# e-c-k-e-r/tortoise-tts

Hardware: AMD Instinct MI355X
Metric: audio-sec/wall-sec (RTF^-1), 16 AR candidates x 80 DDIM steps (higher is better)
Workload: dtype bf16; 1 GPU; configs[1]: 1 utterance/GPU, 64 text tokens, 16 AR candidates x 250 mel tokens (KV-cached decode), latent pass on 16 candidates, 80 DDIM steps with cond-free guidance at T=1088 (11.6 s audio); candidates=16, ddim_steps=80, mel_frames=1088, parallelism=single GPU, small_models=False, vocoder_in_step=False

## Files before the change

### tortoise_tts_amd/csrc/norm.hip

```cpp
#include <stdint.h>

#include "ttk_common.h"
#include "ttk_kernels.h"

namespace ttk {

template <typename OT, int NI>
__global__ void k_layernorm(const float* x, int64_t ldx, int rows, int d, const float* g1, const float* b1,
							const float* g2, const float* b2, OT* out, int64_t ldo, int frag, float* out2, const int64_t* out2_idx, int64_t out2_stride, const int64_t* out2_base) {
	constexpr bool HOIST = NI <= 4;
	const int lane = threadIdx.x & 63;
	const int row = blockIdx.x * (blockDim.x >> 6) + (threadIdx.x >> 6);
	if (row >= rows) return;
	if (out2_base) out2 = (float*)(uintptr_t)out2_base[0];
	if (out2 && out2_idx) out2 += out2_idx[0] * out2_stride;
	const int nchunk = d / 4;
	float4 v[NI];
	float4 pg[HOIST ? 2 : 1][HOIST ? NI : 1], pb[HOIST ? 2 : 1][HOIST ? NI : 1];
#pragma unroll
	for (int i = 0; i < NI; ++i) {
		const int c = lane + 64 * i;
		v[i] = c < nchunk ? *(const float4*)(x + (int64_t)row * ldx + 4 * c) : make_float4(0, 0, 0, 0);
	}
	if (HOIST) {
#pragma unroll
		for (int i = 0; i < (HOIST ? NI : 0); ++i) {
			const int c = lane + 64 * i < nchunk ? lane + 64 * i : 0;
			pg[0][i] = *(const float4*)(g1 + 4 * c); pb[0][i] = *(const float4*)(b1 + 4 * c);
			if (g2) { pg[HOIST ? 1 : 0][i] = *(const float4*)(g2 + 4 * c); pb[HOIST ? 1 : 0][i] = *(const float4*)(b2 + 4 * c); }
		}
	}
#pragma unroll
	for (int pass = 0; pass < 2; ++pass) {
		if (pass == 1 && !g2) break;
		const float* g = pass ? g2 : g1;
		const float* b = pass ? b2 : b1;
		float sum = 0.f;
#pragma unroll
		for (int i = 0; i < NI; ++i) sum += v[i].x + v[i].y + v[i].z + v[i].w;
		const float mean = wave_sum(sum) / (float)d;
		float sq = 0.f;
#pragma unroll
		for (int i = 0; i < NI; ++i)
			if (lane + 64 * i < nchunk) {
				const float a0 = v[i].x - mean, a1 = v[i].y - mean, a2 = v[i].z - mean, a3 = v[i].w - mean;
				sq += a0 * a0 + a1 * a1 + a2 * a2 + a3 * a3;
			}
		const float rstd = rsqrtf(wave_sum(sq) / (float)d + 1e-5f);
#pragma unroll
		for (int i = 0; i < NI; ++i) {
			const int c = lane + 64 * i;
			if (c < nchunk) {
				const float4 gg = HOIST ? pg[HOIST ? pass : 0][HOIST ? i : 0] : *(const float4*)(g + 4 * c), bb = HOIST ? pb[HOIST ? pass : 0][HOIST ? i : 0] : *(const float4*)(b + 4 * c);
				v[i].x = (v[i].x - mean) * rstd * gg.x + bb.x;
				v[i].y = (v[i].y - mean) * rstd * gg.y + bb.y;
				v[i].z = (v[i].z - mean) * rstd * gg.z + bb.z;
				v[i].w = (v[i].w - mean) * rstd * gg.w + bb.w;
			}
		}
	}
#pragma unroll
	for (int i = 0; i < NI; ++i) {
		const int c = lane + 64 * i;
		if (c < nchunk) {
			const int n = 4 * c;
			OT* o = frag ? out + TTK_FRAG_INDEX(row, n, d / 32) : out + (int64_t)row * ldo + n;
			o[0] = (OT)v[i].x; o[1] = (OT)v[i].y; o[2] = (OT)v[i].z; o[3] = (OT)v[i].w;
			if (out2) *(float4*)(out2 + (int64_t)row * d + n) = v[i];
		}
	}
}

void launch_layernorm(int dt, const float* x, int64_t ldx, int rows, int d, const float* g1, const float* b1,
					  const float* g2, const float* b2, void* out, int64_t ldo, int out_f32, hipStream_t s, int frag, float* out2,
					  const int64_t* out2_idx, int64_t out2_stride, const int64_t* out2_base) {
	ProfScope prof(PROF_LAYERNORM, (double)rows * d * (4.0 + (out_f32 ? 4.0 : dtype_size(dt))), s);
	const int grid = (rows + 3) / 4;
#define LN_GO(OT, NI) hipLaunchKernelGGL((k_layernorm<OT, NI>), dim3(grid), dim3(256), 0, s, x, ldx, rows, d, g1, b1, g2, b2, (OT*)out, ldo, frag, out2, out2_idx, out2_stride, out2_base)
	if (out_f32 || dt == DT_F32) { if (d <= 1024) LN_GO(float, 4); else LN_GO(float, 16); }
	else if (dt == DT_F16) { if (d <= 1024) LN_GO(f16, 4); else LN_GO(f16, 16); }
	else { if (d <= 1024) LN_GO(bf16, 4); else LN_GO(bf16, 16); }
#undef LN_GO
}

__global__ __launch_bounds__(256) void k_gn_stats(const float* x, int T, int C, int rows_per_chunk, float* part, const int* tlen, const int* need) {
	const int g = blockIdx.x, b = blockIdx.y, ch = blockIdx.z, cpg = C / 32;
	if (need && !need[b]) return;
	const int Tl = tlen ? tlen[b] : T;
	const int t0 = ch * rows_per_chunk;
	if (t0 >= Tl) return;
	const int rows = min(rows_per_chunk, Tl - t0);
	const float* base = x + ((int64_t)b * T + t0) * C + g * cpg;
	const int n = rows * cpg;
	__shared__ float sh[4];
	float v[8];
	float sum = 0.f;
#pragma unroll
	for (int i = 0; i < 8; ++i) {
		const int e = threadIdx.x + 256 * i;
		const int t = e / cpg, c = e - t * cpg;
		v[i] = e < n ? base[(int64_t)t * C + c] : 0.f;
		sum += v[i];
	}
	sum = wave_sum(sum);
	if ((threadIdx.x & 63) == 0) sh[threadIdx.x >> 6] = sum;
	__syncthreads();
	const float mean = (sh[0] + sh[1] + sh[2] + sh[3]) / (float)n;
	__syncthreads();
	float sq = 0.f;
#pragma unroll
	for (int i = 0; i < 8; ++i)
		if (threadIdx.x + 256 * i < n) { const float d = v[i] - mean; sq += d * d; }
	sq = wave_sum(sq);
	if ((threadIdx.x & 63) == 0) sh[threadIdx.x >> 6] = sq;
	__syncthreads();
	if (threadIdx.x == 0) {
		float* o = part + (((int64_t)b * 32 + g) * gridDim.z + ch) * 3;
		o[0] = (float)n; o[1] = mean; o[2] = sh[0] + sh[1] + sh[2] + sh[3];
	}
}

int gn_rows_per_chunk(int C) { const int r = 2048 / (C / 32); return r < 1 ? 1 : r; }
int gn_num_chunks(int T, int C) { const int r = gn_rows_per_chunk(C); return (T + r - 1) / r; }

void launch_gn_stats(const float* x, int nb, int T, int C, float* part, hipStream_t s, const int* tlen, const int* need) {
	ProfScope prof(PROF_GN_STATS, 4.0 * nb * T * C, s);
	hipLaunchKernelGGL(k_gn_stats, dim3(32, nb, gn_num_chunks(T, C)), dim3(256), 0, s, x, T, C, gn_rows_per_chunk(C), part, tlen, need);
}

template <typename OT>
__global__ __launch_bounds__(256) void k_gn_apply(GnApplyParams p) {
	constexpr int GN_PASSES = 2;
	__shared__ float s_mean[32], s_rstd[32];
	TTK_WSTAMP(p.stamps, blockIdx.x, 0);
	const int c4n = p.C / 4;
	const int rpp = 256 / c4n;
	const int strip = rpp * GN_PASSES;
	const int strips = (p.Tout + strip - 1) / strip;
	const int b = blockIdx.x / strips, t0 = (blockIdx.x - b * strips) * strip;
	const int Tl = p.tlen ? p.tlen[b] : p.Tout;
	const int nch = p.tlen ? (Tl + p.chunk_rows - 1) / p.chunk_rows : p.nchunks;
	const int c = (threadIdx.x % c4n) * 4, rr = threadIdx.x / c4n;
	float4 xv[GN_PASSES];
#pragma unroll
	for (int i = 0; i < GN_PASSES; ++i) {
		const int to = t0 + i * rpp + rr;
		const int ti = to < p.Tout ? (p.row_idx ? p.row_idx[to] : to) : 0;
		xv[i] = *(const float4*)(p.x + ((int64_t)b * p.T + ti) * p.C + c);
	}
	TTK_WSTAMP(p.stamps, blockIdx.x, 1);
	__shared__ unsigned pf_sink[64 * 4];
	if (p.pf)
		l2_touch_for_next(p.pf, p.pf_bytes, p.pf_taps, __builtin_amdgcn_readfirstlane(lds_byte_addr(pf_sink) + (threadIdx.x >> 6) * 256), blockIdx.x, gridDim.x, threadIdx.x, 256);
	{
		const int g = threadIdx.x >> 3, sub = threadIdx.x & 7;
		const float* part = p.ms + ((int64_t)b * 32 + g) * p.nchunks * 3;
		float mean, rstd;
		gn_merge_triples(part, nch, sub, [](const float* q) { return *q; }, mean, rstd);
		if (sub == 0) { s_mean[g] = mean; s_rstd[g] = rstd; }
	}
	__syncthreads();
	TTK_WSTAMP(p.stamps, blockIdx.x, 2);
	const int g = c / (p.C / 32);
	const float mean = s_mean[g], rstd = s_rstd[g];
	const float4 ga = *(const float4*)(p.gamma + c), be = *(const float4*)(p.beta + c);
	float4 sc = make_float4(0.f, 0.f, 0.f, 0.f), sh = sc;
	if (p.scale) { sc = *(const float4*)(p.scale + (int64_t)b * p.ss_stride + c); sh = *(const float4*)(p.shift + (int64_t)b * p.ss_stride + c); }
	float a0, a1, a2, a3, d0, d1, d2, d3;
	gn_fold_coef(mean, rstd, ga.x, be.x, sc.x, sh.x, a0, d0); gn_fold_coef(mean, rstd, ga.y, be.y, sc.y, sh.y, a1, d1);
	gn_fold_coef(mean, rstd, ga.z, be.z, sc.z, sh.z, a2, d2); gn_fold_coef(mean, rstd, ga.w, be.w, sc.w, sh.w, a3, d3);
#pragma unroll
	for (int i = 0; i < GN_PASSES; ++i) {
		const int to = t0 + i * rpp + rr;
		if (to >= p.Tout) continue;
		float o0 = gn_fold_apply(xv[i].x, a0, d0), o1 = gn_fold_apply(xv[i].y, a1, d1), o2 = gn_fold_apply(xv[i].z, a2, d2), o3 = gn_fold_apply(xv[i].w, a3, d3);
		if (p.act == ACT_SILU) { o0 = silu_f(o0); o1 = silu_f(o1); o2 = silu_f(o2); o3 = silu_f(o3); }
		if (to >= Tl) { o0 = 0.f; o1 = 0.f; o2 = 0.f; o3 = 0.f; }
		OT* dst = (OT*)p.out + ((int64_t)b * p.Tout + to) * p.C + c;
		if (sizeof(OT) == 1) {
			*(unsigned*)dst = pack4_fp8(o0, o1, o2, o3);
		} else if (sizeof(OT) == 2) {
			*(uint2*)dst = pack4_16<OT>(o0, o1, o2, o3);
		} else {
			*(float4*)dst = make_float4(o0, o1, o2, o3);
		}
	}
	TTK_WSTAMP(p.stamps, blockIdx.x, 4);
#if defined(TTK_STAMPS) && TTK_STAMPS == 2
	asm volatile("s_waitcnt vmcnt(0)" ::: "memory");
	TTK_WSTAMP(p.stamps, blockIdx.x, 5);
#endif
}

template <typename OT>
__global__ __launch_bounds__(320) void k_gn_apply_c1024(GnApplyParams p) {
	constexpr int C = 1024, GN_PASSES = 4;
	__shared__ unsigned pf_sink[64 * 4];
	TTK_PIN_ARGS(TTK_S(p.x), TTK_S(p.ms), TTK_S(p.gamma), TTK_S(p.beta), TTK_S(p.scale), TTK_S(p.shift), TTK_S(p.ss_stride), TTK_S(p.T), TTK_S(p.nchunks),
				 TTK_S(p.act), TTK_S(p.out), TTK_S(p.tlen), TTK_S(p.chunk_rows), TTK_S(p.pf), TTK_S(p.pf_bytes), TTK_S(p.pf_taps));
	TTK_WSTAMP(p.stamps, blockIdx.y * gridDim.x + blockIdx.x, 0);
	const int tid = threadIdx.x;
	if (tid >= 256) {
		if (p.pf) l2_touch_for_next(p.pf, p.pf_bytes, p.pf_taps, __builtin_amdgcn_readfirstlane(lds_byte_addr(pf_sink)), blockIdx.y * gridDim.x + blockIdx.x,
									gridDim.x * gridDim.y, tid - 256, 64);
		return;
	}
	const int b = blockIdx.y, t0 = blockIdx.x * GN_PASSES;
	const int Tl = p.tlen ? p.tlen[b] : p.T;
	const int nch = p.tlen ? (Tl + p.chunk_rows - 1) / p.chunk_rows : p.nchunks;
	const int c = tid * 4;
	float4 xv[GN_PASSES];
#pragma unroll
	for (int i = 0; i < GN_PASSES; ++i) {
		const int to = t0 + i;
		xv[i] = *(const float4*)(p.x + ((int64_t)b * p.T + (to < p.T ? to : 0)) * C + c);
	}
	const float4 ga = *(const float4*)(p.gamma + c), be = *(const float4*)(p.beta + c);
	float4 sc = make_float4(0.f, 0.f, 0.f, 0.f), sh = sc;
	if (p.scale) { sc = *(const float4*)(p.scale + (int64_t)b * p.ss_stride + c); sh = *(const float4*)(p.shift + (int64_t)b * p.ss_stride + c); }
	TTK_WSTAMP(p.stamps, blockIdx.y * gridDim.x + blockIdx.x, 1);
	float mean, rstd;
	{
		const int g = tid >> 3, sub = tid & 7;
		const float* part = p.ms + ((int64_t)b * 32 + g) * p.nchunks * 3;
		gn_merge_triples(part, nch, sub, [](const float* q) { return *q; }, mean, rstd);
	}
	TTK_WSTAMPD(p.stamps, blockIdx.y * gridDim.x + blockIdx.x, 2, rstd);
	float a0, a1, a2, a3, d0, d1, d2, d3;
	gn_fold_coef(mean, rstd, ga.x, be.x, sc.x, sh.x, a0, d0); gn_fold_coef(mean, rstd, ga.y, be.y, sc.y, sh.y, a1, d1);
	gn_fold_coef(mean, rstd, ga.z, be.z, sc.z, sh.z, a2, d2); gn_fold_coef(mean, rstd, ga.w, be.w, sc.w, sh.w, a3, d3);
#pragma unroll
	for (int i = 0; i < GN_PASSES; ++i) {
		const int to = t0 + i;
		if (to >= p.T) continue;
		float o0 = gn_fold_apply(xv[i].x, a0, d0), o1 = gn_fold_apply(xv[i].y, a1, d1), o2 = gn_fold_apply(xv[i].z, a2, d2), o3 = gn_fold_apply(xv[i].w, a3, d3);
		if (p.act == ACT_SILU) { o0 = silu_f(o0); o1 = silu_f(o1); o2 = silu_f(o2); o3 = silu_f(o3); }
		if (to >= Tl) { o0 = 0.f; o1 = 0.f; o2 = 0.f; o3 = 0.f; }
		OT* dst = (OT*)p.out + ((int64_t)b * p.T + to) * C + c;
		if (sizeof(OT) == 1) *(unsigned*)dst = pack4_fp8(o0, o1, o2, o3);
		else if (sizeof(OT) == 2) *(uint2*)dst = pack4_16<OT>(o0, o1, o2, o3);
		else *(float4*)dst = make_float4(o0, o1, o2, o3);
	}
	TTK_WSTAMP(p.stamps, blockIdx.y * gridDim.x + blockIdx.x, 4);
#if defined(TTK_STAMPS) && TTK_STAMPS == 2
	asm volatile("s_waitcnt vmcnt(0)" ::: "memory");
	TTK_WSTAMP(p.stamps, blockIdx.y * gridDim.x + blockIdx.x, 5);
#endif
}

template <typename OT, int GN_MAXR, int NG = 8>
__global__ __launch_bounds__(320) void k_gn_apply_c1024_even(GnApplyParams p, int q, int rem) {
	constexpr int C = 1024;
	__shared__ unsigned pf_sink[64 * 4];
	TTK_PIN_ARGS(TTK_S(p.x), TTK_S(p.ms), TTK_S(p.gamma), TTK_S(p.beta), TTK_S(p.scale), TTK_S(p.shift), TTK_S(p.ss_stride), TTK_S(p.T), TTK_S(p.nchunks),
				 TTK_S(p.act), TTK_S(p.out), TTK_S(p.pf), TTK_S(p.pf_bytes), TTK_S(p.pf_taps), TTK_S(q), TTK_S(rem));
	TTK_WSTAMP(p.stamps, blockIdx.y * gridDim.x + blockIdx.x, 0);
	const int tid = threadIdx.x;
	if (tid >= 256) {
		if (p.pf) l2_touch_for_next(p.pf, p.pf_bytes, p.pf_taps, __builtin_amdgcn_readfirstlane(lds_byte_addr(pf_sink)), blockIdx.y * gridDim.x + blockIdx.x,
									gridDim.x * gridDim.y, tid - 256, 64);
		return;
	}
	const int b = blockIdx.y, w = blockIdx.x;
	const int t0 = w * q + (w < rem ? w : rem), nrows = q + (w < rem ? 1 : 0);
	const int c = tid * 4;
	float cn[8], cm[8], c2[8];
	gn_load_triples_n<NG>(p.ms + ((int64_t)b * 32 + (tid >> 3)) * p.nchunks * 3, p.nchunks, tid & 7, [](const float* qq) { return *qq; }, cn, cm, c2);
	__builtin_amdgcn_sched_barrier(0);
	float4 xv[GN_MAXR];
#pragma unroll
	for (int i = 0; i < GN_MAXR; ++i) {
		if (NG < 8) xv[i] = *(const float4*)(p.x + ((int64_t)b * p.T + t0 + (i < nrows ? i : nrows - 1)) * C + c);
		else if (i < nrows) xv[i] = *(const float4*)(p.x + ((int64_t)b * p.T + t0 + i) * C + c);
	}
	const float4 ga = *(const float4*)(p.gamma + c), be = *(const float4*)(p.beta + c);
	float4 sc = make_float4(0.f, 0.f, 0.f, 0.f), sh = sc;
	if (NG < 8) {
		const float4 s1 = *(const float4*)((p.scale ? p.scale + (int64_t)b * p.ss_stride : p.gamma) + c), s2 = *(const float4*)((p.scale ? p.shift + (int64_t)b * p.ss_stride : p.beta) + c);
		if (p.scale) { sc = s1; sh = s2; }
	} else if (p.scale) { sc = *(const float4*)(p.scale + (int64_t)b * p.ss_stride + c); sh = *(const float4*)(p.shift + (int64_t)b * p.ss_stride + c); }
	__builtin_amdgcn_sched_barrier(0);
	TTK_WSTAMP(p.stamps, blockIdx.y * gridDim.x + blockIdx.x, 1);
	float mean, rstd;
	gn_merge_loaded(cn, cm, c2, mean, rstd);
	__builtin_amdgcn_sched_barrier(0);
	TTK_WSTAMPD(p.stamps, blockIdx.y * gridDim.x + blockIdx.x, 2, rstd);
	float a0, a1, a2, a3, d0, d1, d2, d3;
	gn_fold_coef(mean, rstd, ga.x, be.x, sc.x, sh.x, a0, d0); gn_fold_coef(mean, rstd, ga.y, be.y, sc.y, sh.y, a1, d1);
	gn_fold_coef(mean, rstd, ga.z, be.z, sc.z, sh.z, a2, d2); gn_fold_coef(mean, rstd, ga.w, be.w, sc.w, sh.w, a3, d3);
#pragma unroll
	for (int i = 0; i < GN_MAXR; ++i) {
		if (i >= nrows) continue;
		float o0 = gn_fold_apply(xv[i].x, a0, d0), o1 = gn_fold_apply(xv[i].y, a1, d1), o2 = gn_fold_apply(xv[i].z, a2, d2), o3 = gn_fold_apply(xv[i].w, a3, d3);
		if (p.act == ACT_SILU) { o0 = silu_f(o0); o1 = silu_f(o1); o2 = silu_f(o2); o3 = silu_f(o3); }
		OT* dst = (OT*)p.out + ((int64_t)b * p.T + t0 + i) * C + c;
		if (sizeof(OT) == 1) *(unsigned*)dst = pack4_fp8(o0, o1, o2, o3);
		else if (sizeof(OT) == 2) *(uint2*)dst = pack4_16<OT>(o0, o1, o2, o3);
		else *(float4*)dst = make_float4(o0, o1, o2, o3);
	}
	TTK_WSTAMP(p.stamps, blockIdx.y * gridDim.x + blockIdx.x, 4);
#if defined(TTK_STAMPS) && TTK_STAMPS == 2
	asm volatile("s_waitcnt vmcnt(0)" ::: "memory");
	TTK_WSTAMP(p.stamps, blockIdx.y * gridDim.x + blockIdx.x, 5);
#endif
}

enum GnApplyForm { GN_GENERIC = 1, GN_STRIPS = 2, GN_EVEN_9 = 3, GN_EVEN_12 = 4, GN_EVEN_18 = 5 };
static int gn_apply_form(const GnApplyParams& p) {
	if (!(p.C == 1024 && !p.row_idx && p.Tout == p.T && p.nb <= 65535)) return GN_GENERIC;
	if (!p.tlen && p.nb >= 1 && p.nb <= 64) {
		const int strips = 256 / p.nb, q = p.T / strips, mr = q + (p.T % strips ? 1 : 0);
		if (q >= 4 && mr <= 18) return p.nchunks <= 24 && mr <= 9 ? GN_EVEN_9 : (p.nchunks <= 24 && mr <= 12 ? GN_EVEN_12 : GN_EVEN_18);
	}
	return GN_STRIPS;
}
const char* gn_apply_form_refusal(const GnApplyParams& p, int form) {
	if (form < 0 || form > GN_EVEN_18) return "form must be 0 (the launcher's choice), 1 (generic), 2 (4-row strips), 3, 4 or 5 (even: 9, 12 or 18 rows)";
	if (form <= GN_GENERIC) return nullptr;
	if (p.C != 1024 || p.row_idx || p.Tout != p.T || p.nb > 65535) return "forms 2 to 5 need C == 1024, no row_idx, Tout == T and nb <= 65535";
	if (form == GN_STRIPS) return nullptr;
	if (p.tlen || p.nb < 1 || p.nb > 64) return "the even forms need no tlen and nb <= 64";
	const int strips = 256 / p.nb, q = p.T / strips, mr = q + (p.T % strips ? 1 : 0);
	if (q < 4 || mr > (form == GN_EVEN_9 ? 9 : (form == GN_EVEN_12 ? 12 : 18))) return "the even forms need strips (T over 256 / nb) of at least 4 rows and at most 9 / 12 / 18";
	if (form != GN_EVEN_18 && p.nchunks > 24) return "forms 3 and 4 read at most 24 statistics chunks";
	return nullptr;
}

template <typename F>
static void gn_out_type(int dt, const GnApplyParams& p, F&& go) {
	if (p.out_f8) go(f8{});
	else if (p.out_f32 || dt == DT_F32) go(float{});
	else if (dt == DT_F16) go(f16{});
	else go(bf16{});
}
void launch_gn_apply(int dt, const GnApplyParams& p, hipStream_t s, int form) {
	ProfScope prof(PROF_GN_APPLY, (double)p.nb * p.Tout * p.C * (4.0 + (p.out_f8 ? 1.0 : p.out_f32 ? 4.0 : dtype_size(dt))), s);
	if (!form) form = gn_apply_form(p);
	gn_out_type(dt, p, [&](auto ot) {
		using OT = decltype(ot);
		if (form == GN_GENERIC) {
			const int strip = (256 / (p.C / 4)) * 2;
			hipLaunchKernelGGL((k_gn_apply<OT>), dim3(p.nb * ((p.Tout + strip - 1) / strip)), dim3(256), 0, s, p);
		} else if (form == GN_STRIPS) {
			hipLaunchKernelGGL((k_gn_apply_c1024<OT>), dim3((p.T + 3) / 4, p.nb), dim3(320), 0, s, p);
		} else {
			const int strips = 256 / p.nb, q = p.T / strips, rem = p.T % strips;
			const dim3 grid(strips, p.nb);
			if (form == GN_EVEN_9) hipLaunchKernelGGL((k_gn_apply_c1024_even<OT, 9, 3>), grid, dim3(320), 0, s, p, q, rem);
			else if (form == GN_EVEN_12) hipLaunchKernelGGL((k_gn_apply_c1024_even<OT, 12, 3>), grid, dim3(320), 0, s, p, q, rem);
			else hipLaunchKernelGGL((k_gn_apply_c1024_even<OT, 18, 8>), grid, dim3(320), 0, s, p, q, rem);
		}
	});
}

}
```

### tortoise_tts_amd/csrc/gemv.hip

```cpp
#include <hip/hip_ext.h>

#include "ttk_common.h"
#include "ttk_kernels.h"
#include "ttk_rng.h"

namespace ttk {

template <typename T> __device__ __forceinline__ void fold_stats(const typename Frag<T>::type& a, float& s1, float& s2) {
#pragma unroll
	for (int j = 0; j < 8; ++j) { const float f = (float)a[j]; s1 += f; s2 = fmaf(f, f, s2); }
}
template <> __device__ __forceinline__ void fold_stats<bf16>(const bf16x8& a, float& s1, float& s2) {
	typedef __bf16 bf16x2 __attribute__((ext_vector_type(2)));
	const bf16x2 one = {(bf16)1.0f, (bf16)1.0f};
#pragma unroll
	for (int j = 0; j < 8; j += 2) {
		const bf16x2 x = {a[j], a[j + 1]};
		s2 = __builtin_amdgcn_fdot2_f32_bf16(x, x, s2, false);
		s1 = __builtin_amdgcn_fdot2_f32_bf16(x, one, s1, false);
	}
}
template <> __device__ __forceinline__ void fold_stats<f16>(const f16x8& a, float& s1, float& s2) {
	typedef _Float16 f16x2 __attribute__((ext_vector_type(2)));
	const f16x2 one = {(f16)1.0f, (f16)1.0f};
#pragma unroll
	for (int j = 0; j < 8; j += 2) {
		const f16x2 x = {a[j], a[j + 1]};
		s2 = __builtin_amdgcn_fdot2(x, x, s2, false);
		s1 = __builtin_amdgcn_fdot2(x, one, s1, false);
	}
}

template <typename T, int MT, int ROLE, int NW, int KPW, bool W8>
__global__ __launch_bounds__(64 * NW) void k_gemv(GemvParams p) {
	typedef typename Frag<T>::type FragT;
	typedef WFrag<T, W8> WF;
	typedef typename WF::raw WRaw;
	constexpr int ES = sizeof(T);
	constexpr bool FOLD = ROLE == GV_QKV || ROLE == GV_FC;
	constexpr bool NARROW = ROLE == GV_PROJ;
	constexpr int KS = NW * KPW;
	extern __shared__ __attribute__((aligned(16))) float gv_red[];
	float* red = gv_red;
	float* rstat = red + NW * MT * 64 * 4;
	asm volatile("" :: "s"(p.Wp), "s"(p.a), "s"(p.bias), "s"(p.csum), "s"(p.out_f32), "s"(p.out_T), "s"(p.qbuf), "s"(p.kcache), "s"(p.vcache),
				 "s"(p.d_pos), "s"(p.noise), "s"(p.rng), "s"(p.draws), "s"(p.health), "s"(p.M), "s"(p.N), "s"(p.max_ctx), "s"(p.H), "s"(p.row0), "s"(p.q_scale), "s"(p.wscale));
	TTK_WSTAMP(p.stamps, blockIdx.x, 0);
	const int tid = threadIdx.x, lane = tid & 63, wave = tid >> 6;
	int nt, sub = 0;
	if (NARROW) { const int b = blockIdx.x; nt = ((b >> 5) << 3) + (b & 7); sub = (b >> 3) & 3; }
	else nt = blockIdx.x;

	const int l2 = lane, r = wave & 3;
	const int n = NARROW ? nt * 16 + 4 * sub + (l2 & 3) : nt * 16 + (l2 & 15);
	const bool mine = tid < 256 && (!NARROW || (l2 & 15) < 4) && n < p.N;
	const int nn = n < p.N ? n : p.N - 1;
	float bias = 0.f, fcs = 0.f, res[MT];
	RngArgs rng = {};
	int64_t draw[MT];
	int kv_pos = 0;
	if (ROLE == GV_QKV) kv_pos = *p.d_pos;
	if (ROLE == GV_HEAD && p.d_pos && blockIdx.x == 0 && tid == 0) *(int*)p.d_pos += 1;
	const bool noise = ROLE == GV_HEAD && p.noise != nullptr;
	if (p.bias) bias = p.bias[nn];
	if (FOLD) fcs = p.csum[nn];
	if (noise) rng = *(const RngArgs*)p.rng;
#pragma unroll
	for (int mt = 0; mt < MT; ++mt) {
		res[mt] = 0.f; draw[mt] = 0;
		int m = mt * 16 + 4 * (l2 >> 4) + r;
		m = m < p.M ? m : p.M - 1;
		if (ROLE == GV_PROJ) res[mt] = p.out_f32[(int64_t)m * p.N + nn];
		if (noise) draw[mt] = p.draws[m];
	}

	constexpr int OPREGS = (MT + 1) * (ES == 4 ? 8 : 4);
	constexpr int PRE0 = 64 / OPREGS >= 8 ? 8 : (64 / OPREGS >= 4 ? 4 : (64 / OPREGS >= 2 ? 2 : 1));
	constexpr int PRE = PRE0 < KPW ? PRE0 : KPW;
	static_assert(KPW % PRE == 0, "k-steps per wave must be a multiple of the operand batch");
	const int ks0 = wave * KPW;
	const WRaw* wp = (const WRaw*)p.Wp + ((int64_t)nt * KS + ks0) * 64 + (NARROW ? ((lane & ~15) | (4 * sub + (lane & 3))) : lane);
	const FragT* ap = (const FragT*)p.a + (int64_t)ks0 * 64 + lane;
	f32x4 acc[MT];
	float fs1[MT], fs2[MT];
#pragma unroll
	for (int mt = 0; mt < MT; ++mt) { acc[mt] = f32x4{0.f, 0.f, 0.f, 0.f}; fs1[mt] = 0.f; fs2[mt] = 0.f; }
	constexpr bool WLDS = NARROW && ES == 2;
	if constexpr (WLDS) {
		static_assert(KPW % 4 == 0, "dense weight requests cover four k-steps");
		constexpr int WL = KPW / 4;
		WRaw* wl = (WRaw*)(rstat) + wave * (KPW * 16);
		const WRaw* wd = (const WRaw*)p.Wp + ((int64_t)nt * KS + ks0 + (lane >> 4)) * 64 + ((lane >> 2) & 3) * 16 + 4 * sub + (lane & 3);
		WRaw wq[WL];
#pragma unroll
		for (int i = 0; i < WL; ++i) wq[i] = TTK_WLOAD(wd + i * 4 * 64);
		FragT a0[PRE][MT];
#pragma unroll
		for (int u = 0; u < PRE; ++u)
#pragma unroll
			for (int mt = 0; mt < MT; ++mt) a0[u][mt] = ap[((int64_t)mt * KS + u) * 64];
		TTK_WSTAMP(p.stamps, blockIdx.x, 2);
		__builtin_amdgcn_sched_barrier(0);
#pragma unroll
		for (int i = 0; i < WL; ++i) wl[i * 64 + lane] = wq[i];
		const int rd = ((lane >> 4) << 2) + (lane & 3);
#pragma unroll
		for (int kb = 0; kb < KPW; kb += PRE) {
			FragT a[PRE][MT];
			if (kb + PRE < KPW) {
#pragma unroll
				for (int u = 0; u < PRE; ++u)
#pragma unroll
					for (int mt = 0; mt < MT; ++mt) a[u][mt] = ap[((int64_t)mt * KS + kb + PRE + u) * 64];
			}
			__builtin_amdgcn_sched_barrier(0);
#pragma unroll
			for (int u = 0; u < PRE; ++u) {
				const WRaw b = wl[(kb + u) * 16 + rd];
#pragma unroll
				for (int mt = 0; mt < MT; ++mt) acc[mt] = mma16<T>(a0[u][mt], WF::dec(b), acc[mt]);
			}
			if (kb + PRE < KPW) {
#pragma unroll
				for (int u = 0; u < PRE; ++u)
#pragma unroll
					for (int mt = 0; mt < MT; ++mt) a0[u][mt] = a[u][mt];
			}
		}
	} else {
#pragma unroll
	for (int kb = 0; kb < KPW; kb += PRE) {
		WRaw b[PRE];
		FragT a[PRE][MT];
#pragma unroll
		for (int u = 0; u < PRE; ++u) {
			b[u] = TTK_WLOAD(wp + (kb + u) * 64);
#pragma unroll
			for (int mt = 0; mt < MT; ++mt) a[u][mt] = ap[((int64_t)mt * KS + kb + u) * 64];
		}
		if (kb == 0) TTK_WSTAMP(p.stamps, blockIdx.x, 2);
		__builtin_amdgcn_sched_barrier(0);
#pragma unroll
		for (int u = 0; u < PRE; ++u)
#pragma unroll
			for (int mt = 0; mt < MT; ++mt) {
				if (FOLD) fold_stats<T>(a[u][mt], fs1[mt], fs2[mt]);
				acc[mt] = mma16<T>(a[u][mt], WF::dec(b[u]), acc[mt]);
			}
	}
	}
	if (FOLD) {
#pragma unroll
		for (int mt = 0; mt < MT; ++mt) {
			fs1[mt] = fold16_add(fs1[mt]); fs2[mt] = fold16_add(fs2[mt]);
			fs1[mt] = fold32_add(fs1[mt]); fs2[mt] = fold32_add(fs2[mt]);
			if (lane < 16) *(float2*)(rstat + ((wave * MT + mt) * 16 + lane) * 2) = make_float2(fs1[mt], fs2[mt]);
		}
	}
	TTK_WSTAMPD(p.stamps, blockIdx.x, 3, acc[0][0]);
#pragma unroll
	for (int mt = 0; mt < MT; ++mt) *(f32x4*)(red + ((wave * MT + mt) * 64 + lane) * 4) = acc[mt];
	__syncthreads();
	TTK_WSTAMP(p.stamps, blockIdx.x, 4);
	if (!mine) return;
#pragma unroll
	for (int mt = 0; mt < MT; ++mt) {
		const int m = mt * 16 + 4 * (l2 >> 4) + r;
		if (m >= p.M) continue;
		float vs = 0.f;
#pragma unroll
		for (int w = 0; w < NW; ++w) vs += red[((w * MT + mt) * 64 + l2) * 4 + r];
		float v;
		if (FOLD) {
			float a1 = 0.f, a2 = 0.f;
#pragma unroll
			for (int w = 0; w < NW; ++w) { const float2 t = *(const float2*)(rstat + ((w * MT + mt) * 16 + 4 * (l2 >> 4) + r) * 2); a1 += t.x; a2 += t.y; }
			const float mean = a1 / (float)(32 * KS);
			const float var = fmaxf(fmaf(-mean, mean, a2 / (float)(32 * KS)), 0.f);
			const float rstd = rsqrtf(var + 1e-5f);
			v = (vs - mean * fcs) * rstd + bias;
			if (p.health && blockIdx.x == 0 && (l2 & 15) == 0) {
				const int bad = (mean * mean > 64.f * (var + 1e-5f) ? 1 : 0) | (a2 - a2 != 0.f ? 2 : 0);
				if (bad) atomicOr(p.health, bad);
			}
		} else {
			v = (W8 ? vs * p.wscale : vs) + bias;
		}
		if (ROLE == GV_HEAD) {
			p.out_f32[(int64_t)m * p.N + n] = v;
			if (noise) {
				int mrow = p.row0 + m;
				const int grp = (int)rng.group;
				if (grp > 0) while (mrow >= grp) mrow -= grp;
				p.noise[(int64_t)m * p.N + n] = torch_exponential_at(rng, draw[mt], (rng.row0 + mrow) * (int64_t)p.N + n);
			}
		} else if (ROLE == GV_PROJ) {
			p.out_f32[(int64_t)m * p.N + n] = res[mt] + v;
			if (p.out_T) ((T*)p.out_T)[TTK_FRAG_INDEX(m, n, p.N >> 5)] = cvt<T>(res[mt] + v);
		} else if (ROLE == GV_FC) {
			((T*)p.out_T)[TTK_FRAG_INDEX(m, n, p.N >> 5)] = cvt<T>(gelu_new_f(v));
		} else {
			constexpr int d = 32 * KS;
			const int which = n / d, c = n - which * d;
			if (which == 0) {
				p.qbuf[(int64_t)m * d + c] = v * p.q_scale;
			} else {
				const int h = c >> 6, dd = c & 63;
				T* cache = (T*)(which == 1 ? p.kcache : p.vcache);
				if (kv_pos < p.max_ctx) cache[(((int64_t)m * p.H + h) * p.max_ctx + kv_pos) * 64 + dd] = cvt<T>(v);
			}
		}
	}
	TTK_WSTAMP(p.stamps, blockIdx.x, 5);
#if defined(TTK_STAMPS) && TTK_STAMPS == 2
	asm volatile("s_waitcnt vmcnt(0)" ::: "memory");
	TTK_WSTAMP(p.stamps, blockIdx.x, 6);
#endif
}

template <typename T, int MT, int ROLE, int NW, int KPW, bool W8>
static void gemv_go(const GemvParams& p, hipStream_t s, hipEvent_t ea, hipEvent_t eb) {
	constexpr bool FOLD = ROLE == GV_QKV || ROLE == GV_FC;
	const int tiles = (p.N + 15) / 16;
	const int grid = ROLE == GV_PROJ ? tiles * 4 : tiles;
	const size_t lds = (size_t)NW * MT * 64 * 4 * sizeof(float) + (FOLD ? (size_t)NW * MT * 16 * 2 * sizeof(float) : 0)
					   + (ROLE == GV_PROJ && sizeof(T) == 2 ? (size_t)NW * KPW * 16 * (W8 ? 8 : 16) : 0);
	hipExtLaunchKernelGGL((k_gemv<T, MT, ROLE, NW, KPW, W8>), dim3(grid), dim3(64 * NW), (unsigned)lds, s, ea, eb, 0, p);
}

template <typename T, int ROLE, int NW, int KPW, bool W8>
static void gemv_mt(const GemvParams& p, hipStream_t s, hipEvent_t ea, hipEvent_t eb) {
	const int mt = decode_row_tiles(p.M);
	if (mt == 1) gemv_go<T, 1, ROLE, NW, KPW, W8>(p, s, ea, eb);
	else if (mt == 2) gemv_go<T, 2, ROLE, NW, KPW, W8>(p, s, ea, eb);
	else if (mt == 3 && sizeof(T) == 2) gemv_go<T, sizeof(T) == 2 ? 3 : 2, ROLE, NW, KPW, W8>(p, s, ea, eb);
	else if (sizeof(T) == 2) gemv_go<T, sizeof(T) == 2 ? 4 : 2, ROLE, NW, KPW, W8>(p, s, ea, eb);
}

template <typename T, int ROLE, bool W8>
static bool gemv_role(const GemvParams& p, hipStream_t s, hipEvent_t ea, hipEvent_t eb) {
	constexpr bool F32 = sizeof(T) == 4;
	if (ROLE == GV_HEAD) {
		if (p.K != 1024) return false;
		gemv_mt<T, ROLE, 4, 8, W8>(p, s, ea, eb);
	} else if (p.K == 1024) {
		gemv_mt<T, ROLE, F32 ? 8 : 4, F32 ? 4 : 8, W8>(p, s, ea, eb);
	} else if (p.K == 4096 && ROLE == GV_PROJ) {
		gemv_mt<T, ROLE, 8, 16, W8>(p, s, ea, eb);
	} else {
		return false;
	}
	return true;
}

bool gemv_supported(int dt, int role, const GemvParams& p) {
	if (dt != DT_BF16 && dt != DT_F16 && dt != DT_F32) return false;
	if (p.M < 1 || p.M > (dt == DT_F32 ? 32 : 64)) return false;
	if (p.w8 && (dt != DT_BF16 || role != GV_PROJ)) return false;
	if (role == GV_HEAD) return p.K == 1024;
	if (role == GV_PROJ) return (p.K == 1024 || p.K == 4096) && p.N % 128 == 0;
	if (role == GV_QKV) return p.K == 1024 && p.N == 3 * p.K;
	return p.K == 1024 && p.N % 32 == 0;
}

bool launch_gemv(int dt, int role, const GemvParams& p, hipStream_t s) {
	if (!gemv_supported(dt, role, p)) return false;
	hipEvent_t ea = nullptr, eb = nullptr;
	if (g_prof_on) prof_pair(PROF_SKINNY, (double)p.N * p.K * (p.w8 ? 1 : dtype_size(dt)) + 4.0 * p.N + 4.0 * p.M * p.K + 4.0 * p.M * p.N, &ea, &eb);
#define GV_DISPATCH(T, W8) \
	(role == GV_QKV ? gemv_role<T, GV_QKV, false>(p, s, ea, eb) : role == GV_FC ? gemv_role<T, GV_FC, false>(p, s, ea, eb) : \
	 role == GV_HEAD ? gemv_role<T, GV_HEAD, false>(p, s, ea, eb) : gemv_role<T, GV_PROJ, W8>(p, s, ea, eb))
	if (dt == DT_BF16) return p.w8 ? GV_DISPATCH(bf16, true) : GV_DISPATCH(bf16, false);
	if (dt == DT_F16) return GV_DISPATCH(f16, false);
	return GV_DISPATCH(float, false);
#undef GV_DISPATCH
}

}
```

Baseline: 40.78 audio-sec/wall-sec.

## Slice GroupNorm apply by channel per XCD for L2 locality

When 32 is divisible by the batch count, the even-strip GroupNorm apply kernel switches to a 1-D grid of 256 blocks. Each block's low three index bits pick a fixed 128-channel slice, which lines it up with the round-robin XCD assignment. The rest of the block index selects batch and time strip, and each block covers eight times as many rows using a strided row mapping. The aim is for each XCD's L2 to see only its own channel slice of gamma, beta, scale/shift and group statistics. The cost is narrower 512-byte row segments per access, and a compile-time macro can turn the path off.

```diff
diff --git a/tortoise_tts_amd/csrc/norm.hip b/tortoise_tts_amd/csrc/norm.hip
--- a/tortoise_tts_amd/csrc/norm.hip
+++ b/tortoise_tts_amd/csrc/norm.hip
@@ -4,6 +4,10 @@
 #include "ttk_kernels.h"
 
 namespace ttk {
+
+#ifndef TTK_GN_XCD_SLICE
+#define TTK_GN_XCD_SLICE 1
+#endif
 
 template <typename OT, int NI>
 __global__ void k_layernorm(const float* x, int64_t ldx, int rows, int d, const float* g1, const float* b1,
@@ -248,12 +252,12 @@
 #endif
 }
 
-template <typename OT, int GN_MAXR, int NG = 8>
-__global__ __launch_bounds__(320) void k_gn_apply_c1024_even(GnApplyParams p, int q, int rem) {
+template <typename OT, int GN_MAXR, int NG = 8, bool SLICE = false>
+__global__ __launch_bounds__(320) void k_gn_apply_c1024_even(GnApplyParams p, int q, int rem, int rsh) {
 	constexpr int C = 1024;
 	__shared__ unsigned pf_sink[64 * 4];
 	TTK_PIN_ARGS(TTK_S(p.x), TTK_S(p.ms), TTK_S(p.gamma), TTK_S(p.beta), TTK_S(p.scale), TTK_S(p.shift), TTK_S(p.ss_stride), TTK_S(p.T), TTK_S(p.nchunks),
-				 TTK_S(p.act), TTK_S(p.out), TTK_S(p.pf), TTK_S(p.pf_bytes), TTK_S(p.pf_taps), TTK_S(q), TTK_S(rem));
+				 TTK_S(p.act), TTK_S(p.out), TTK_S(p.pf), TTK_S(p.pf_bytes), TTK_S(p.pf_taps), TTK_S(q), TTK_S(rem), TTK_S(rsh));
 	TTK_WSTAMP(p.stamps, blockIdx.y * gridDim.x + blockIdx.x, 0);
 	const int tid = threadIdx.x;
 	if (tid >= 256) {
@@ -261,17 +265,22 @@
 									gridDim.x * gridDim.y, tid - 256, 64);
 		return;
 	}
-	const int b = blockIdx.y, w = blockIdx.x;
+	const int xcd = blockIdx.x & 7, rank = blockIdx.x >> 3;
+	const int b = SLICE ? rank >> rsh : blockIdx.y, w = SLICE ? rank & ((1 << rsh) - 1) : blockIdx.x;
 	const int t0 = w * q + (w < rem ? w : rem), nrows = q + (w < rem ? 1 : 0);
-	const int c = tid * 4;
+	const int c = SLICE ? 128 * xcd + (tid & 31) * 4 : tid * 4;
+	const int r0 = SLICE ? tid >> 5 : 0;
+	constexpr int RS = SLICE ? 8 : 1;
+	const int g = SLICE ? 4 * xcd + ((tid & 31) >> 3) : tid >> 3;
 	float cn[8], cm[8], c2[8];
-	gn_load_triples_n<NG>(p.ms + ((int64_t)b * 32 + (tid >> 3)) * p.nchunks * 3, p.nchunks, tid & 7, [](const float* qq) { return *qq; }, cn, cm, c2);
+	gn_load_triples_n<NG>(p.ms + ((int64_t)b * 32 + g) * p.nchunks * 3, p.nchunks, tid & 7, [](const float* qq) { return *qq; }, cn, cm, c2);
 	__builtin_amdgcn_sched_barrier(0);
 	float4 xv[GN_MAXR];
 #pragma unroll
 	for (int i = 0; i < GN_MAXR; ++i) {
-		if (NG < 8) xv[i] = *(const float4*)(p.x + ((int64_t)b * p.T + t0 + (i < nrows ? i : nrows - 1)) * C + c);
-		else if (i < nrows) xv[i] = *(const float4*)(p.x + ((int64_t)b * p.T + t0 + i) * C + c);
+		const int r = r0 + RS * i;
+		if (NG < 8) xv[i] = *(const float4*)(p.x + ((int64_t)b * p.T + t0 + (r < nrows ? r : nrows - 1)) * C + c);
+		else if (r < nrows) xv[i] = *(const float4*)(p.x + ((int64_t)b * p.T + t0 + r) * C + c);
 	}
 	const float4 ga = *(const float4*)(p.gamma + c), be = *(const float4*)(p.beta + c);
 	float4 sc = make_float4(0.f, 0.f, 0.f, 0.f), sh = sc;
@@ -290,10 +299,11 @@
 	gn_fold_coef(mean, rstd, ga.z, be.z, sc.z, sh.z, a2, d2); gn_fold_coef(mean, rstd, ga.w, be.w, sc.w, sh.w, a3, d3);
 #pragma unroll
 	for (int i = 0; i < GN_MAXR; ++i) {
-		if (i >= nrows) continue;
+		const int r = r0 + RS * i;
+		if (r >= nrows) continue;
 		float o0 = gn_fold_apply(xv[i].x, a0, d0), o1 = gn_fold_apply(xv[i].y, a1, d1), o2 = gn_fold_apply(xv[i].z, a2, d2), o3 = gn_fold_apply(xv[i].w, a3, d3);
 		if (p.act == ACT_SILU) { o0 = silu_f(o0); o1 = silu_f(o1); o2 = silu_f(o2); o3 = silu_f(o3); }
-		OT* dst = (OT*)p.out + ((int64_t)b * p.T + t0 + i) * C + c;
+		OT* dst = (OT*)p.out + ((int64_t)b * p.T + t0 + r) * C + c;
 		if (sizeof(OT) == 1) *(unsigned*)dst = pack4_fp8(o0, o1, o2, o3);
 		else if (sizeof(OT) == 2) *(uint2*)dst = pack4_16<OT>(o0, o1, o2, o3);
 		else *(float4*)dst = make_float4(o0, o1, o2, o3);
@@ -344,11 +354,15 @@
 		} else if (form == GN_STRIPS) {
 			hipLaunchKernelGGL((k_gn_apply_c1024<OT>), dim3((p.T + 3) / 4, p.nb), dim3(320), 0, s, p);
 		} else {
-			const int strips = 256 / p.nb, q = p.T / strips, rem = p.T % strips;
-			const dim3 grid(strips, p.nb);
-			if (form == GN_EVEN_9) hipLaunchKernelGGL((k_gn_apply_c1024_even<OT, 9, 3>), grid, dim3(320), 0, s, p, q, rem);
-			else if (form == GN_EVEN_12) hipLaunchKernelGGL((k_gn_apply_c1024_even<OT, 12, 3>), grid, dim3(320), 0, s, p, q, rem);
-			else hipLaunchKernelGGL((k_gn_apply_c1024_even<OT, 18, 8>), grid, dim3(320), 0, s, p, q, rem);
+			const bool slice = TTK_GN_XCD_SLICE && 32 % p.nb == 0;
+			const int strips = slice ? 32 / p.nb : 256 / p.nb, q = p.T / strips, rem = p.T % strips, rsh = slice ? __builtin_ctz(strips) : 0;
+			const dim3 grid = slice ? dim3(256) : dim3(strips, p.nb);
+#define GN_EVEN_GO(MAXR, NGR) do { if (slice) hipLaunchKernelGGL((k_gn_apply_c1024_even<OT, MAXR, NGR, true>), grid, dim3(320), 0, s, p, q, rem, rsh); \
+								   else hipLaunchKernelGGL((k_gn_apply_c1024_even<OT, MAXR, NGR, false>), grid, dim3(320), 0, s, p, q, rem, rsh); } while (0)
+			if (form == GN_EVEN_9) GN_EVEN_GO(9, 3);
+			else if (form == GN_EVEN_12) GN_EVEN_GO(12, 3);
+			else GN_EVEN_GO(18, 8);
+#undef GN_EVEN_GO
 		}
 	});
 }
```

Result: no change. 40.77 audio-sec/wall-sec (-0.0%).

## Software-pipeline gemv operand loads with register-budgeted multi-set prefetch

Applied to the files above, without the earlier changes.

Replaces the fixed operand batch size in the decode gemv kernel with a register-budget-driven batch and a ring of NSET operand sets. Loads for later k-batches are issued while earlier batches feed the MFMAs, so memory latency overlaps with compute in both the LDS-weight and direct-weight paths. The role dispatch is also made constexpr so unused template instantiations are not generated. It costs extra registers, which may reduce occupancy or cause spills if the budget estimate is off.

```diff
diff --git a/tortoise_tts_amd/csrc/gemv.hip b/tortoise_tts_amd/csrc/gemv.hip
--- a/tortoise_tts_amd/csrc/gemv.hip
+++ b/tortoise_tts_amd/csrc/gemv.hip
@@ -31,6 +31,17 @@
 	}
 }
 
+constexpr int gv_budget(int nw) { return nw <= 4 ? 160 : 96; }
+constexpr int gv_batch(int kpw, int step, int fixed, int nw) {
+	if (kpw * step + fixed <= gv_budget(nw)) return kpw;
+	int pre = 1;
+	while (2 * pre < kpw && 2 * (2 * pre) * step + fixed <= gv_budget(nw)) pre *= 2;
+	return pre;
+}
+constexpr int gv_sets(int kpw, int pre, int step, int fixed, int nw) {
+	const int fit = (gv_budget(nw) - fixed) / (pre * step), nb = kpw / pre;
+	return fit < nb ? (fit < 1 ? 1 : fit) : nb;
+}
 template <typename T, int MT, int ROLE, int NW, int KPW, bool W8>
 __global__ __launch_bounds__(64 * NW) void k_gemv(GemvParams p) {
 	typedef typename Frag<T>::type FragT;
@@ -74,10 +85,12 @@
 		if (noise) draw[mt] = p.draws[m];
 	}
 
-	constexpr int OPREGS = (MT + 1) * (ES == 4 ? 8 : 4);
-	constexpr int PRE0 = 64 / OPREGS >= 8 ? 8 : (64 / OPREGS >= 4 ? 4 : (64 / OPREGS >= 2 ? 2 : 1));
-	constexpr int PRE = PRE0 < KPW ? PRE0 : KPW;
-	static_assert(KPW % PRE == 0, "k-steps per wave must be a multiple of the operand batch");
+	constexpr bool WLDS = NARROW && ES == 2;
+	constexpr int STEP = MT * (int)(sizeof(FragT) / 4) + (WLDS ? 0 : (int)(sizeof(WRaw) / 4));
+	constexpr int FIXED = WLDS ? KPW / 4 * (int)(sizeof(WRaw) / 4) : 0;
+	constexpr int PRE = gv_batch(KPW, STEP, FIXED, NW);
+	constexpr int NB = KPW / PRE, NSET = gv_sets(KPW, PRE, STEP, FIXED, NW);
+	static_assert(KPW % PRE == 0 && (NB == 1 || NSET >= 2) && NSET * PRE * STEP + FIXED <= gv_budget(NW), "operand batches must tile the wave's k-steps inside the budget");
 	const int ks0 = wave * KPW;
 	const WRaw* wp = (const WRaw*)p.Wp + ((int64_t)nt * KS + ks0) * 64 + (NARROW ? ((lane & ~15) | (4 * sub + (lane & 3))) : lane);
 	const FragT* ap = (const FragT*)p.a + (int64_t)ks0 * 64 + lane;
@@ -85,7 +98,7 @@
 	float fs1[MT], fs2[MT];
 #pragma unroll
 	for (int mt = 0; mt < MT; ++mt) { acc[mt] = f32x4{0.f, 0.f, 0.f, 0.f}; fs1[mt] = 0.f; fs2[mt] = 0.f; }
-	constexpr bool WLDS = NARROW && ES == 2;
+	FragT a[NSET][PRE][MT];
 	if constexpr (WLDS) {
 		static_assert(KPW % 4 == 0, "dense weight requests cover four k-steps");
 		constexpr int WL = KPW / 4;
@@ -94,60 +107,69 @@
 		WRaw wq[WL];
 #pragma unroll
 		for (int i = 0; i < WL; ++i) wq[i] = TTK_WLOAD(wd + i * 4 * 64);
-		FragT a0[PRE][MT];
-#pragma unroll
-		for (int u = 0; u < PRE; ++u)
-#pragma unroll
-			for (int mt = 0; mt < MT; ++mt) a0[u][mt] = ap[((int64_t)mt * KS + u) * 64];
+		__builtin_amdgcn_sched_barrier(0);
+#pragma unroll
+		for (int s = 0; s < NSET; ++s)
+#pragma unroll
+			for (int u = 0; u < PRE; ++u) {
+#pragma unroll
+				for (int mt = 0; mt < MT; ++mt) a[s][u][mt] = ap[((int64_t)mt * KS + s * PRE + u) * 64];
+				__builtin_amdgcn_sched_barrier(0);
+			}
 		TTK_WSTAMP(p.stamps, blockIdx.x, 2);
 		__builtin_amdgcn_sched_barrier(0);
 #pragma unroll
 		for (int i = 0; i < WL; ++i) wl[i * 64 + lane] = wq[i];
 		const int rd = ((lane >> 4) << 2) + (lane & 3);
 #pragma unroll
-		for (int kb = 0; kb < KPW; kb += PRE) {
-			FragT a[PRE][MT];
-			if (kb + PRE < KPW) {
+		for (int bi = 0; bi < NB; ++bi) {
+#pragma unroll
+			for (int u = 0; u < PRE; ++u) {
+				const WRaw b = wl[(bi * PRE + u) * 16 + rd];
+#pragma unroll
+				for (int mt = 0; mt < MT; ++mt) acc[mt] = mma16<T>(a[bi % NSET][u][mt], WF::dec(b), acc[mt]);
+			}
+			__builtin_amdgcn_sched_barrier(0);
+			if (bi + NSET < NB) {
 #pragma unroll
 				for (int u = 0; u < PRE; ++u)
 #pragma unroll
-					for (int mt = 0; mt < MT; ++mt) a[u][mt] = ap[((int64_t)mt * KS + kb + PRE + u) * 64];
-			}
+					for (int mt = 0; mt < MT; ++mt) a[bi % NSET][u][mt] = ap[((int64_t)mt * KS + (bi + NSET) * PRE + u) * 64];
+				__builtin_amdgcn_sched_barrier(0);
+			}
+		}
+	} else {
+		WRaw b[NSET][PRE];
+#pragma unroll
+		for (int s = 0; s < NSET; ++s)
+#pragma unroll
+			for (int u = 0; u < PRE; ++u) {
+				b[s][u] = TTK_WLOAD(wp + (s * PRE + u) * 64);
+#pragma unroll
+				for (int mt = 0; mt < MT; ++mt) a[s][u][mt] = ap[((int64_t)mt * KS + s * PRE + u) * 64];
+			}
+		TTK_WSTAMP(p.stamps, blockIdx.x, 2);
+		__builtin_amdgcn_sched_barrier(0);
+#pragma unroll
+		for (int bi = 0; bi < NB; ++bi) {
+#pragma unroll
+			for (int u = 0; u < PRE; ++u)
+#pragma unroll
+				for (int mt = 0; mt < MT; ++mt) {
+					if (FOLD) fold_stats<T>(a[bi % NSET][u][mt], fs1[mt], fs2[mt]);
+					acc[mt] = mma16<T>(a[bi % NSET][u][mt], WF::dec(b[bi % NSET][u]), acc[mt]);
+				}
 			__builtin_amdgcn_sched_barrier(0);
-#pragma unroll
-			for (int u = 0; u < PRE; ++u) {
-				const WRaw b = wl[(kb + u) * 16 + rd];
-#pragma unroll
-				for (int mt = 0; mt < MT; ++mt) acc[mt] = mma16<T>(a0[u][mt], WF::dec(b), acc[mt]);
-			}
-			if (kb + PRE < KPW) {
-#pragma unroll
-				for (int u = 0; u < PRE; ++u)
-#pragma unroll
-					for (int mt = 0; mt < MT; ++mt) a0[u][mt] = a[u][mt];
-			}
-		}
-	} else {
-#pragma unroll
-	for (int kb = 0; kb < KPW; kb += PRE) {
-		WRaw b[PRE];
-		FragT a[PRE][MT];
-#pragma unroll
-		for (int u = 0; u < PRE; ++u) {
-			b[u] = TTK_WLOAD(wp + (kb + u) * 64);
-#pragma unroll
-			for (int mt = 0; mt < MT; ++mt) a[u][mt] = ap[((int64_t)mt * KS + kb + u) * 64];
-		}
-		if (kb == 0) TTK_WSTAMP(p.stamps, blockIdx.x, 2);
-		__builtin_amdgcn_sched_barrier(0);
-#pragma unroll
-		for (int u = 0; u < PRE; ++u)
-#pragma unroll
-			for (int mt = 0; mt < MT; ++mt) {
-				if (FOLD) fold_stats<T>(a[u][mt], fs1[mt], fs2[mt]);
-				acc[mt] = mma16<T>(a[u][mt], WF::dec(b[u]), acc[mt]);
-			}
-	}
+			if (bi + NSET < NB) {
+#pragma unroll
+				for (int u = 0; u < PRE; ++u) {
+					b[bi % NSET][u] = TTK_WLOAD(wp + ((bi + NSET) * PRE + u) * 64);
+#pragma unroll
+					for (int mt = 0; mt < MT; ++mt) a[bi % NSET][u][mt] = ap[((int64_t)mt * KS + (bi + NSET) * PRE + u) * 64];
+				}
+				__builtin_amdgcn_sched_barrier(0);
+			}
+		}
 	}
 	if (FOLD) {
 #pragma unroll
@@ -240,17 +262,23 @@
 template <typename T, int ROLE, bool W8>
 static bool gemv_role(const GemvParams& p, hipStream_t s, hipEvent_t ea, hipEvent_t eb) {
 	constexpr bool F32 = sizeof(T) == 4;
-	if (ROLE == GV_HEAD) {
+	if constexpr (ROLE == GV_HEAD) {
 		if (p.K != 1024) return false;
 		gemv_mt<T, ROLE, 4, 8, W8>(p, s, ea, eb);
-	} else if (p.K == 1024) {
-		gemv_mt<T, ROLE, F32 ? 8 : 4, F32 ? 4 : 8, W8>(p, s, ea, eb);
-	} else if (p.K == 4096 && ROLE == GV_PROJ) {
-		gemv_mt<T, ROLE, 8, 16, W8>(p, s, ea, eb);
+		return true;
 	} else {
+		if (p.K == 1024) {
+			gemv_mt<T, ROLE, F32 ? 8 : 4, F32 ? 4 : 8, W8>(p, s, ea, eb);
+			return true;
+		}
+		if constexpr (ROLE == GV_PROJ) {
+			if (p.K == 4096) {
+				gemv_mt<T, ROLE, 8, 16, W8>(p, s, ea, eb);
+				return true;
+			}
+		}
 		return false;
 	}
-	return true;
 }
 
 bool gemv_supported(int dt, int role, const GemvParams& p) {
```

Result: no change. 40.85 audio-sec/wall-sec before, 40.87 audio-sec/wall-sec after, median of 4 (+0.0%).
